# Unalome81/IEEE-802.11-OFDM-QPSK-Simulator

Hardware: AMD Instinct MI355X
Metric: OFDM symbols/sec (whole node) over BER-vs-SNR sweep; achieved HBM GB/s vs peak (higher is better)
Workload: dtype f32

## Files before the change

### ieee-802.11-ofdm-qpsk-simulator_amd/csrc/ofdm_rxcommon.h

```cpp
#pragma once
#include "ofdm_internal.h"

namespace ofdm {

struct TxSignSrc { uint32_t re, im; };
__host__ __device__ constexpr TxSignSrc tx_sign_src(const uint32_t (&w)[3], int m) {
    const uint32_t wd = w[(2 * m) >> 5];
    const int sh = (2 * m) & 31;
    return {(wd ^ (wd << 1)) << sh, wd << sh};
}
__host__ __device__ constexpr int tx_sign_tbl(int conv, int bin) { return (conv == OFDM_CONV_C && (bin & 1)) ? 0xD2 : 0x78; }
__host__ __device__ constexpr uint32_t bitop3_ref(uint32_t a, uint32_t b, uint32_t c, int tbl) {
    uint32_t o = 0u;
    for (int i = 0; i < 32; ++i) {
        const uint32_t idx = (((a >> i) & 1u) << 2) | (((b >> i) & 1u) << 1) | ((c >> i) & 1u);
        o |= (((uint32_t)tbl >> idx) & 1u) << i;
    }
    return o;
}
template <int CONV>
__host__ __device__ constexpr bool tx_sign_map_is_d10() {
    for (int bin = 0; bin < 64; ++bin) {
        const int m = data_index(bin);
        if (m < 0) continue;
// ... 127 lines not shown
struct SymState {
    float evm_pre;
    uint32_t be, ax;
    uint32_t d[3];
};

__device__ __forceinline__ void sym_init(SymState &st) {
    st.evm_pre = 0.f; st.be = 0u; st.ax = 0u; st.d[0] = st.d[1] = st.d[2] = 0u;
}
template <int KIND>
__device__ __forceinline__ float finish_evm(const SymState &st) { return KIND == 2 ? 4.0f * st.evm_pre : st.evm_pre; }

__device__ __forceinline__ uint32_t dbl_u32(uint32_t t) {
    uint32_t r;
    asm("v_add_u32_e32 %0, %1, %1" : "=v"(r) : "v"(t));
    return r;
}

template <bool DUMP, int R, int KIND, typename HF>
__device__ __forceinline__ void demap_sub(const float2 (&x)[64], uint32_t t, HF &&Hof, float2 *dump_eq, SymState &st) {
    uint32_t sm;
    asm volatile("v_mov_b32 %0, 0x80000000" : "=v"(sm));
    constexpr float cd = KIND == 2 ? 0.5f * INV_SQRT2 : INV_SQRT2;
    uint32_t em = 0u;
    static_for<0, 16>([&](auto kc) {
        constexpr int bin = 4 * decltype(kc)::value + R;
        constexpr int m = data_index(bin);
        if constexpr (m >= 0) {
            const EqOut<KIND> e = Hof(x[digit_rev4(bin)], std::integral_constant<int, bin>{});
            const uint32_t ti = t, tr = dbl_u32(t);
            t = dbl_u32(tr);
            const uint32_t ur = __builtin_amdgcn_bitop3_b32(__float_as_uint(e.u.x), tr, sm, 0x78);
            const uint32_t ui = __builtin_amdgcn_bitop3_b32(__float_as_uint(e.u.y), ti, sm, 0x78);
            float ex, ey;
            if constexpr (KIND == 0) {
                ex = __uint_as_float(ur) - cd;
                ey = __uint_as_float(ui) - cd;
            } else {
                ex = fmaf(__uint_as_float(ur), e.r, -cd);
                ey = fmaf(__uint_as_float(ui), e.r, -cd);
            }
            st.evm_pre = fmaf(ex, ex, fmaf(ey, ey, st.evm_pre));
            em = __builtin_amdgcn_alignbit(em, ur, 31);
            em = __builtin_amdgcn_alignbit(em, ui, 31);
            if constexpr (DUMP) {
                const float g = KIND == 0 ? 1.0f : KIND == 1 ? e.r : 2.0f * e.r;
                const float2 z = KIND == 0 ? e.u : make_float2(e.u.x * g, e.u.y * g);
                if (dump_eq) dump_eq[m] = z;
                const uint32_t pr = z.x > 0.f, pi = z.y > 0.f;
                constexpr int wi = (2 * m) >> 5;
                constexpr int s0 = 31 - ((2 * m) & 31), s1 = 31 - ((2 * m + 1) & 31);
                st.d[wi] |= ((pi ^ 1u) << s0) | ((pr ^ pi) << s1);
            }
        }
    });
    opaque(st.evm_pre);
    st.ax += __popc(em);
    st.be += __popc(em & 0x55555555u) + __popc((em ^ (em >> 1)) & 0x55555555u);
}

template <int BIN>
__device__ __forceinline__ EqOut<2> ls_equalise(float2 Y) {
    const float2 S = dpp_c<DPP_QUAD_BCAST0>(Y);
    EqOut<2> e;
    e.r = __builtin_amdgcn_rcpf(fmaf(S.x, S.x, S.y * S.y));
    e.u = cscale(cmulc(Y, S), (float)ltf_sign(BIN));
    return e;
}

template <typename F>
struct EqFn {
    F f;
    template <int R>
    __device__ __forceinline__ void prefetch(const float2 (&)[64]) {}
    template <typename B>
    __device__ __forceinline__ auto operator()(float2 Y, B b) { return f(Y, b); }
};
template <typename F>
__device__ __forceinline__ EqFn<F> eq_fn(F f) { return EqFn<F>{f}; }

struct FrameAcc {
    uint64_t errs = 0, frames = 0;
    int64_t pre_q = 0, dbpre_q = 0, dbpost_q = 0;
};

__device__ __forceinline__ int64_t q20_nonneg(float x) {
    const float v = __builtin_rintf(x * (float)OFDM_EVM_Q_SCALE);
    const float hi = __builtin_floorf(v * 0x1p-32f);
    const uint32_t lo = (uint32_t)fmaf(hi, -0x1p32f, v);
    return (int64_t)(((uint64_t)(uint32_t)hi << 32) | lo);
}
__device__ __forceinline__ int64_t q20_db(float db) {
    return (int64_t)(int32_t)__builtin_rintf(db * (float)OFDM_EVM_Q_SCALE);
}

__device__ __forceinline__ void frame_metrics(FrameAcc &acc, float fe_pre, uint32_t ferr, uint32_t fax) {
    constexpr float K = 3.01029995663981195214f, L96 = 6.58496250072115618146f;
    acc.errs = (uint64_t)ferr | ((uint64_t)fax << 32);
    acc.frames = (uint64_t)(ferr > 0u) | ((uint64_t)(fax > 0u) << 32);
    acc.pre_q = q20_nonneg(fe_pre);
    const float lg = K * (__builtin_amdgcn_logf(fe_pre) - L96);
    acc.dbpre_q = q20_db(fe_pre > 0.f ? fmaxf(lg, -400.0f) : -400.0f);
    acc.dbpost_q = fax > 0u ? q20_db(K * (__builtin_amdgcn_logf((float)fax) + (1.0f - L96))) : 0;
}

__device__ __forceinline__ void flush_lanes(const FrameAcc &acc, bool leader, unsigned long long *slots ) {
    if (leader) {
        atomicAdd(&slots[0], (unsigned long long)acc.errs);
        atomicAdd(&slots[1], (unsigned long long)acc.frames);
        atomicAdd(&slots[2], (unsigned long long)acc.pre_q);
        atomicAdd(&slots[3], (unsigned long long)acc.dbpre_q);
        atomicAdd(&slots[4], (unsigned long long)acc.dbpost_q);
    }
}

__device__ __forceinline__ int slot_term(const unsigned long long *s, int k, unsigned long long &v) {
    switch (k) {
        case 0: v = s[0] & 0xffffffffull; return OFDM_C_BIT_ERR;
        case 1: v = s[0] >> 32; return OFDM_C_EVM_POST_AXIS;
        case 2: v = s[1] & 0xffffffffull; return OFDM_C_FRAME_ERR;
        case 3: v = s[1] >> 32; return OFDM_C_EVMDB_POST_FINITE;
        case 4: v = s[2]; return OFDM_C_EVM_PRE_Q;
        case 5: v = s[3]; return OFDM_C_EVMDB_PRE_Q;
        default: v = s[4]; return OFDM_C_EVMDB_POST_Q;
    }
}

template <int S>
__device__ __forceinline__ void block_flush(const RxArgs &a, unsigned long long (*sacc)[S], int tid) {
    __syncthreads();
    for (int i = tid; i < a.n_snr * 7; i += blockDim.x) {
        const int q = i / 7, k = i % 7;
        unsigned long long v;
        const int ci = slot_term(sacc[q], k, v);
        if (v) atomicAdd(&a.counters[q * OFDM_NCOUNTERS + ci], v);
    }
    if (blockIdx.x == 0) {
        for (int q = tid; q < a.n_snr; q += blockDim.x) {
            unsigned long long *c = a.counters + q * OFDM_NCOUNTERS;
            atomicAdd(&c[OFDM_C_FRAMES], (unsigned long long)a.n_frames);
            atomicAdd(&c[OFDM_C_SYMBOLS], (unsigned long long)(2 * a.n_frames));
            atomicAdd(&c[OFDM_C_BITS], (unsigned long long)(192 * a.n_frames));
            atomicAdd(&c[OFDM_C_EVM_TERMS], (unsigned long long)(96 * a.n_frames));
        }
    }
}
template <int S>
__device__ __forceinline__ void block_flush(const RxArgs &a, unsigned long long (*sacc)[S]) {
    block_flush(a, sacc, (int)threadIdx.x);
}



template <int CONV, typename TA>
__device__ __forceinline__ void tx_symbol(const TA &a, int64_t sidx) {
    const uint64_t s = a.first_symbol + (uint64_t)sidx;
    uint32_t w[3];
    if (a.payload == OFDM_PAYLOAD_RANDOM) {
        const uint4 o = philox10((uint32_t)s, (uint32_t)(s >> 32), 0u, STREAM_BITS, a.k0, a.k1);
        w[0] = o.x; w[1] = o.y; w[2] = o.z;
    } else {
        const int r = (int)(s % (uint64_t)a.table_frames);
        w[0] = a.table[3 * r]; w[1] = a.table[3 * r + 1]; w[2] = a.table[3 * r + 2];
    }
    float2 X[64];
    static_for<0, 4>([&](auto gc) {
        constexpr int g = decltype(gc)::value;
        uint32_t wg[3] = {w[0], w[1], w[2]};
        opaque(wg[0]); opaque(wg[1]); opaque(wg[2]);
        static_for<0, 16>([&](auto pc) {
            constexpr int i = 16 * (decltype(pc)::value >> 2) + 4 * g + (decltype(pc)::value & 3);
            X[i] = tx_bin<CONV, i>(wg);
        });
        static_for<0, 4>([&](auto ic) { dif_stage1<true, 4 * g + decltype(ic)::value>(X); });
        sched_fence();
    });
    const uint32_t so = (uint32_t)sidx;
    [[maybe_unused]] const int64_t P = a.pitch;
    static_for<0, 4>([&](auto rc) {
        constexpr int R = decltype(rc)::value;
        dif_sub16<true, R>(X);
        static_for<0, 16>([&](auto nc) {
            constexpr int n = 4 * decltype(nc)::value + R;
            const float2 v = cscale(X[digit_rev4(n)], (n & 1) ? -1.0f / 64.0f : 1.0f / 64.0f);
            gst((gf2 *)(a.tx + (16 + n) * P), so, v);
            if constexpr (n >= 48) gst((gf2 *)(a.tx + (n - 48) * P), so, v);
        });
        sched_fence();
    });
    a.bits[so] = w[0];
    a.bits[P + so] = w[1];
    a.bits[2 * P + so] = w[2];
    a.bits[3 * P + so] = demap_word<0>(w);
    a.bits[4 * P + so] = demap_word<1>(w);
    a.bits[5 * P + so] = demap_word<2>(w);
    a.bits[6 * P + so] = demap_word<3>(w);
    uint32_t pw[3];
    pair_words(w, pw);
    a.bits[7 * P + so] = pw[0];
    a.bits[8 * P + so] = pw[1];
    a.bits[9 * P + so] = pw[2];
}

}
```

### ieee-802.11-ofdm-qpsk-simulator_amd/csrc/ofdm_rxpack.hip

```cpp
#include "ofdm_internal.h"
#include "ofdm_rxcommon.h"

#define OFDM_RX_PACK_WAVES 2
#define OFDM_RX_PACK_IDEAL_WAVES 3

namespace ofdm {

constexpr int PK_FRAMES = 64;
constexpr int PK_SYMS = 2 * PK_FRAMES;

typedef float f4v __attribute__((ext_vector_type(4)));
typedef __attribute__((address_space(3))) const f4v lcf4;
typedef unsigned int u2v __attribute__((ext_vector_type(2)));
typedef __attribute__((address_space(3))) const u2v lcu2;
typedef __attribute__((address_space(3))) f2v lf2;

constexpr int PACK_PF = 2;
constexpr int PACK_GEN_SPLIT = 2;
constexpr int PACK_FENCE_PAIRS = 2;

__host__ __device__ constexpr int rev16(int m) { return ((m & 3) << 2) | (m >> 2); }
__host__ __device__ constexpr int pos32(int k) { return (k & 1) ? 16 + rev16(k >> 1) : rev16(k >> 1); }

template <int K>
__device__ __forceinline__ float2 chan_bin(const float2 (&h)[4]) {
    float2 H = h[0];
    H = csub(H, twiddle<K * 1, false>(h[1]));
    H = cadd(H, twiddle<K * 2, false>(h[2]));
    return csub(H, twiddle<K * 3, false>(h[3]));
}

template <int HALF>
__device__ __forceinline__ void chan_pairs(const float2 (&h)[4], float4 *col) {
    static_for<12 * HALF, 12 * HALF + 12>([&](auto pc) {
        constexpr int p = decltype(pc)::value;
        constexpr int k = pair_bin(p);
        const float2 Hk = chan_bin<k>(h), Hm = chan_bin<64 - k>(h);
        col[p * PK_FRAMES] = make_float4(Hk.x, Hk.y, Hm.x, Hm.y);
        sched_fence();
    });
}

__device__ __forceinline__ void clean_spectrum(const RxArgs &a, int64_t s, float4 *spec_col ) {
    gcf2 *src = (gcf2 *)(a.tx + 16 * a.pitch + s);
    int P = (int)a.pitch;
    opaque(P);
    float2 x[64];
    static_for<0, 4>([&](auto gc) {
        constexpr int g = decltype(gc)::value;
        gcf2 *sp = src;
        opaque(sp);
        static_for<0, 16>([&](auto pc) {
            constexpr int n = 16 * (decltype(pc)::value >> 2) + 4 * g + (decltype(pc)::value & 3);
            const float2 v = gld(sp, n * P);
            x[n] = (n & 1) ? make_float2(-v.x, -v.y) : v;
        });
        static_for<0, 4>([&](auto ic) { dif_stage1<false, 4 * g + decltype(ic)::value>(x); });
        sched_fence();
    });
    auto store = [&](auto pc) {
        constexpr int p = decltype(pc)::value;
        constexpr int k = pair_bin(p);
        const float2 c0 = x[digit_rev4(k)], c1 = x[digit_rev4(64 - k)];
        spec_col[p * 2 * PK_FRAMES] = make_float4(c0.x, c0.y, c1.x, c1.y);
    };
    static_for<0, 4>([&](auto rc) { dif_sub16<false, decltype(rc)::value>(x); });
    static_for<0, PACK_PAIRS>(store);
}

template <int KIND, bool DUMP, bool WALK, int TBL>
__device__ __forceinline__ void demap_bin(float2 u, float r, uint32_t &t, float sx, float sy, uint32_t sm, float &evm,
                                          uint32_t &em, int m, float2 *dump_eq, uint32_t (&dbits)[3]) {
    constexpr float cd = KIND == 2 ? 0.5f * INV_SQRT2 : INV_SQRT2;
    uint32_t ur, ui;
    if constexpr (WALK) {
        const uint32_t ti = t, tr = dbl_u32(t);
        t = dbl_u32(tr);
        ur = __builtin_amdgcn_bitop3_b32(__float_as_uint(u.x), tr, sm, 0x78);
        ui = __builtin_amdgcn_bitop3_b32(__float_as_uint(u.y), ti, sm, 0x78);
    } else {
        ur = __builtin_amdgcn_bitop3_b32(__float_as_uint(u.x), __float_as_uint(sx), sm, TBL);
        ui = __builtin_amdgcn_bitop3_b32(__float_as_uint(u.y), __float_as_uint(sy), sm, TBL);
    }
    float ex, ey;
    if constexpr (KIND == 0) {
        ex = __uint_as_float(ur) - cd;
        ey = __uint_as_float(ui) - cd;
    } else {
        ex = fmaf(__uint_as_float(ur), r, -cd);
        ey = fmaf(__uint_as_float(ui), r, -cd);
    }
    evm = fmaf(ex, ex, fmaf(ey, ey, evm));
    em = __builtin_amdgcn_alignbit(em, ur, 31);
    em = __builtin_amdgcn_alignbit(em, ui, 31);
    if constexpr (DUMP) {
        const float g = KIND == 0 ? 1.0f : 2.0f * r;
        const float2 z = make_float2(u.x * g, u.y * g);
        if (dump_eq) dump_eq[m] = z;
        const uint32_t pr = z.x > 0.f, pi = z.y > 0.f;
        const int wi = (2 * m) >> 5, s0 = 31 - ((2 * m) & 31), s1 = 31 - ((2 * m + 1) & 31);
        dbits[wi] |= ((pi ^ 1u) << s0) | ((pr ^ pi) << s1);
    }
}

template <typename KS>
__device__ __forceinline__ Noise4 pack_noise(const PhiloxHead &hd, uint32_t c2, const KS &keys, uint32_t k1, float K) {
    uint4 o;
    if constexpr (std::is_same_v<KS, PhiloxKeysV>) o = philox10_c2(hd, c2, keys);
    else o = philox10_c2(hd, c2, keys, k1);
    return noise4_of(o, K);
}

typedef unsigned int u4v __attribute__((ext_vector_type(4)));
static_assert(sizeof(PhiloxWords) == sizeof(u4v), "one 16-byte read per block");
typedef __attribute__((address_space(3))) const u4v cwords;
__device__ __forceinline__ Noise4 pack_noise(const PhiloxMid &md, cwords *w, uint32_t k0, uint32_t k1, float K) {
    const u4v v = *w;
    return noise4_of(philox10_c2(md, v.x, v.y, v.z, k0, k1), K);
}
__device__ __forceinline__ Noise4 pack_noise(const PhiloxMid &md, lcu2 *w, lcu2 *q, uint32_t k0, uint32_t k1, float K) {
    const u2v v = *w, u = *q;
    return noise4_of(philox10_c2(md, v.x, v.y, u.x, u.y, k0, k1), K);
}

#ifdef OFDM_PACK_STAMPS
#include <cstdio>
static __device__ unsigned long long g_pack_stamps[4][8];
#define PK_STAMP(k)                                                                  \
    do {                                                                             \
        const unsigned long long t_ = __builtin_amdgcn_s_memtime();                  \
        st_acc[k] += t_ - st_t;                                                      \
        st_t = t_;                                                                   \
    } while (0)
#else
#define PK_STAMP(k) do { } while (0)
#endif

#define OFDM_RX_PACK_FADE_WAVES 2
#define PACK_SACC_SUB_LS 4
#define PACK_SACC_SUB 1
template <int KIND, int CONV, int CHAN, bool DUMP>
__global__ __launch_bounds__(256, KIND == 2 ? (CHAN == OFDM_CHAN_RAYLEIGH4 ? OFDM_RX_PACK_FADE_WAVES : OFDM_RX_PACK_WAVES)
                                            : OFDM_RX_PACK_IDEAL_WAVES) void rx_pack_kernel(RxArgs a) {
    constexpr bool FADE = CHAN == OFDM_CHAN_RAYLEIGH4;
    static_assert(!FADE || KIND == 2, "the packed Rayleigh receiver is the LS one");
    constexpr bool WLATE = KIND == 2 && !FADE;
    constexpr bool QW = KIND == 2 && !FADE;
    __shared__ __attribute__((aligned(16))) float4 spec[PACK_PAIRS][2][PK_FRAMES];
    __shared__ __attribute__((aligned(16))) float4 ce[PACK_PAIRS];
    __shared__ __attribute__((aligned(16))) float4 fce[FADE ? PACK_PAIRS : 1][FADE ? PK_FRAMES : 1];
    __shared__ __attribute__((aligned(8))) uint32_t truth[FADE ? 3 : 1][FADE ? PK_SYMS : 2];
    constexpr int SUBN = KIND != 2 ? PACK_SACC_SUB : FADE ? (PACK_SACC_SUB_LS < 4 ? PACK_SACC_SUB_LS : 4)
                                                      : PACK_SACC_SUB_LS;
    constexpr int SACC_XQ = 16;
    __shared__ unsigned long long sacc[OFDM_MAX_SNR][5];
    __shared__ unsigned long long sacx[SUBN > 1 ? SACC_XQ : 1][SUBN > 1 ? 5 * (SUBN - 1) : 1];
    auto slots = [&](int q, int ln) -> unsigned long long * {
        const int c = ln % SUBN;
        return SUBN > 1 && c > 0 && q < SACC_XQ ? &sacx[q][5 * (c - 1)] : sacc[q];
    };
    __shared__ __attribute__((aligned(16))) std::conditional_t<QW, u2v, u4v> wlds[PACK_BLOCKS];
    __shared__ __attribute__((aligned(8))) u2v qw[QW ? PACK_BLOCKS : 1][QW ? PK_FRAMES : 1];
    __shared__ uint32_t pf_dummy[64];
    __shared__ __attribute__((aligned(8))) float2 lds_keep[1];
    const int tid = threadIdx.x, lane = tid & 63;
    const int wv = __builtin_amdgcn_readfirstlane(tid >> 6);
#ifdef OFDM_PACK_STAMPS
    unsigned long long st_acc[8] = {0, 0, 0, 0, 0, 0, 0, 0};
    unsigned long long st_t = __builtin_amdgcn_s_memtime();
#endif
    for (int i = tid; i < a.n_snr * 5; i += blockDim.x) (&sacc[0][0])[i] = 0ull;
    if constexpr (SUBN > 1)
        for (int i = tid; i < SACC_XQ * 5 * (SUBN - 1); i += blockDim.x) (&sacx[0][0])[i] = 0ull;
    if constexpr (KIND == 2) {
        if (wv == 0) {
            float2 x[64];
            static_for<0, 64>([&](auto nc) {
                constexpr int n = decltype(nc)::value;
                const float2 v = a.ltf[n];
                x[n] = (n & 1) ? make_float2(-2.0f * v.x, -2.0f * v.y) : make_float2(2.0f * v.x, 2.0f * v.y);
            });
            fft64<false>(x);
            if (lane == 0) {
                static_for<0, PACK_PAIRS>([&](auto pc) {
                    constexpr int p = decltype(pc)::value;
                    constexpr int k = pair_bin(p);
                    const float2 c0 = x[digit_rev4(k)], c1 = x[digit_rev4(64 - k)];
                    ce[p] = make_float4(c0.x, c0.y, c1.x, c1.y);
                });
            }
        }
    }
    const int64_t n_groups = (a.n_frames + PK_FRAMES - 1) / PK_FRAMES;
    const int B = (int)gridDim.x, G = (int)n_groups, R = G / B, T = G - R * B;
    const int S = T > 0 ? max(1, min(4, B / T)) : 1;
    const int n_items = R * B + T * S;
    __shared__ int next_item;
    for (int w = blockIdx.x; w < n_items; w = __builtin_amdgcn_readfirstlane(next_item)) {
        const bool tail = w >= R * B;
        const int tw = tail ? w - R * B : 0;
        const int64_t grp = tail ? R * B + tw / S : w;
        const int sub = tail ? tw % S : 0, ns = tail ? S : 1;
        __syncthreads();
        PK_STAMP(0);
        const uint64_t fg = a.first_frame + (uint64_t)(grp * PK_FRAMES);
        const uint32_t row = (uint32_t)(fg >> 32) - (uint32_t)(a.first_frame >> 32);
        const bool uniform_hi = (uint32_t)((fg + (PK_FRAMES - 1)) >> 32) == (uint32_t)(fg >> 32) && row < 2u;
        int t = tid;
        opaque(t);
        if constexpr (QW) {
            if (uniform_hi) {
                const uint32_t flo = (uint32_t)fg + (uint32_t)(t & 63);
                const int s0 = (PACK_BLOCKS / 4) * wv;
#pragma unroll
                for (int i = 0; i < PACK_BLOCKS / 4; ++i) {
                    const uint2 qv = philox_qword(flo, a.philox_words[row * PACK_BLOCKS + s0 + i].y, a.k0);
                    u2v o; o.x = qv.x; o.y = qv.y;
                    qw[s0 + i][t & 63] = o;
                }
            }
        }
        using KArgs = const __attribute__((address_space(4))) RxArgs;
        KArgs *ap = (KArgs *)__builtin_amdgcn_kernarg_segment_ptr();
        asm volatile("" : "+s"(ap));
        const bool own_tx = ap->own.n_sym > 0;
        if (own_tx) {
            if (t >= PK_SYMS) {
                const int64_t sidx = grp * PK_SYMS + (t - PK_SYMS);
                if (sidx < ap->own.n_sym) {
                    if (ap->own_conv == OFDM_CONV_C) tx_symbol<OFDM_CONV_C>(ap->own, sidx);
                    else tx_symbol<OFDM_CONV_MATLAB>(ap->own, sidx);
                }
            }
            __syncthreads();
        }
        if (t < PK_SYMS) {
            clean_spectrum(a, grp * PK_SYMS + t, &spec[0][t & 1][t >> 1]);
        } else {
            const int j = t - PK_SYMS;
            if constexpr (FADE) {
                const uint32_t *src = a.bits + 7 * a.pitch + grp * PK_SYMS + j;
                truth[0][j] = src[0];
                truth[1][j] = src[a.pitch];
                truth[2][j] = src[2 * a.pitch];
            }
            if (j < 64) {
                int nx = 0;
                if (j == 0) nx = B + (int)atomicAdd(a.work, 1ull);
                nx = __builtin_amdgcn_readlane(nx, 0);
                if (j == 0) next_item = nx;
                if (nx < n_items && !own_tx && !WLATE) {
                    const int64_t ng = nx < R * B ? nx : R * B + (nx - R * B) / S;
#pragma unroll
                    for (int i = 0; i < 8; ++i) {
                        const int line = j + 64 * i;
                        const float2 *p = a.tx + (int64_t)(16 + (line >> 3)) * a.pitch + ng * PK_SYMS + (line & 7) * 16;
                        __builtin_amdgcn_global_load_lds((__attribute__((address_space(1))) void *)p,
                                                         (__attribute__((address_space(3))) void *)pf_dummy, 4, 0, 0);
                    }
                }
            }
            if (ap->nx.n_sym > 0 && sub == 0) {
                for (int64_t sidx = grp * PK_SYMS + j; sidx < ap->nx.n_sym; sidx += (int64_t)G * PK_SYMS) {
                    if (ap->nx_conv == OFDM_CONV_C) tx_symbol<OFDM_CONV_C>(ap->nx, sidx);
                    else tx_symbol<OFDM_CONV_MATLAB>(ap->nx, sidx);
                }
            }
            if (uniform_hi && j >= 64 && j < 64 + PACK_BLOCKS) {
                const u4v v = ((const u4v *)a.philox_words)[row * PACK_BLOCKS + (j - 64)];
                if constexpr (QW) { u2v o; o.x = v.x; o.y = v.z; wlds[j - 64] = o; }
                else wlds[j - 64] = v;
            }
            if constexpr (FADE) {
                const int fr = j & 63;
                const uint64_t ff = a.first_frame + (uint64_t)(grp * PK_FRAMES + fr);
                float2 h[4];
                channel_taps((uint32_t)ff, (uint32_t)(ff >> 32), a.k0, a.k1, h);
                if (j < 64) chan_pairs<0>(h, &fce[0][fr]);
                else chan_pairs<1>(h, &fce[0][fr]);
            }
        }
        PK_STAMP(1);
        __syncthreads();
        PK_STAMP(2);
        if constexpr (FADE) {
            for (int it = t; it < PACK_PAIRS * PK_FRAMES; it += 256) {
                const int p = it >> 6, fr = it & 63;
                const float4 H = fce[p][fr], c0 = spec[p][0][fr], c1 = spec[p][1][fr], e = ce[p];
                const float2 Hk = make_float2(H.x, H.y), Hm = make_float2(H.z, H.w);
                float2 u = cmul(Hk, make_float2(c0.x, c0.y)), v = cmul(Hm, make_float2(c0.z, c0.w));
                spec[p][0][fr] = make_float4(u.x, u.y, v.x, v.y);
                u = cmul(Hk, make_float2(c1.x, c1.y)); v = cmul(Hm, make_float2(c1.z, c1.w));
                spec[p][1][fr] = make_float4(u.x, u.y, v.x, v.y);
                u = cmul(Hk, make_float2(e.x, e.y)); v = cmul(Hm, make_float2(e.z, e.w));
                fce[p][fr] = make_float4(u.x, u.y, v.x, v.y);
            }
            __syncthreads();
        }
        PK_STAMP(3);
        const int64_t fl = grp * PK_FRAMES + lane;
        const bool valid = fl < a.n_frames;
        const uint64_t f = a.first_frame + (uint64_t)fl;
        auto snr_loop = [&](auto fastc) __attribute__((always_inline)) {
        constexpr bool FAST = decltype(fastc)::value;
        using WordsP = std::conditional_t<QW, lcu2, cwords> *;
        WordsP wtab = (WordsP)&wlds[0];
        for (int q = wv + 4 * sub; q < a.n_snr; q += 4 * ns) {
            if constexpr (WLATE) {
                if (wv == 2 && q + 4 * ns >= a.n_snr) {
                    const int nx = __builtin_amdgcn_readfirstlane(next_item);
                    using KArgsW = const __attribute__((address_space(4))) RxArgs;
                    KArgsW *apw = (KArgsW *)__builtin_amdgcn_kernarg_segment_ptr();
                    if (nx < n_items && apw->own.n_sym == 0) {
                        const int64_t ng = nx < R * B ? nx : R * B + (nx - R * B) / S;
                        int ln = lane;
                        opaque(ln);
#pragma unroll
                        for (int i = 0; i < 8; ++i) {
                            const int line = ln + 64 * i;
                            const float2 *p = a.tx + (int64_t)(16 + (line >> 3)) * a.pitch + ng * PK_SYMS + (line & 7) * 16;
                            __builtin_amdgcn_global_load_lds((__attribute__((address_space(1))) void *)p,
                                                             (__attribute__((address_space(3))) void *)pf_dummy, 4, 0, 0);
                        }
                    }
                }
            }
            uint32_t flo = (uint32_t)f, fhi = (uint32_t)(f >> 32);
            opaque(flo); opaque(fhi);
            const float sigma = a.sigma[q];
            const uint32_t qs = STREAM_NOISE | (uint32_t)(a.q_base + q);
            const PhiloxHead hd = philox_head(flo, fhi, qs, a.k1);
            const PhiloxMid md = philox_mid(hd);
            WordsP wt = wtab;
            lcu2 *qp = (lcu2 *)&qw[0][QW ? lane : 0];
            auto noise = [&](uint32_t blk, int slot, float Kn) __attribute__((always_inline)) {
                if constexpr (FAST && QW) return pack_noise(md, (lcu2 *)(wt + slot), qp + slot * PK_FRAMES, a.k0, a.k1, Kn);
                else if constexpr (FAST) return pack_noise(md, (cwords *)(wt + slot), a.k0, a.k1, Kn);
                else return pack_noise(hd, blk, a.k0, a.k1, Kn);
            };
            float2 z[64];
            float2 ee[PACK_PAIRS];
            lf2 *keep = (lf2 *)&lds_keep[0];
            opaque(keep);
            if constexpr (KIND == 2) {
                const float KE = noise_k(sigma * 1.41421356237309504880f);
                static_for<0, 4>([&](auto ic) {
                    constexpr int i = decltype(ic)::value;
                    uint32_t tg = 48u + 2 * i;
                    if constexpr (FAST) opaque(wt);
                    else opaque(tg);
                    if constexpr (FAST && QW) opaque(qp);
                    static_for<0, 2>([&](auto hc) {
                        constexpr int h = decltype(hc)::value;
                        const Noise4 lo = noise(tg + h, 2 * i + h, KE);
                        const Noise4 hi = noise(tg + 8 + h, 2 * i + 8 + h, KE);
                        constexpr int m = 4 * i + 2 * h;
                        z[m] = make_float2(lo.r0 * lo.c0, -(lo.r0 * lo.s0));
                        z[m + 1] = make_float2(lo.r1 * lo.c1, -(lo.r1 * lo.s1));
                        z[m + 16] = make_float2(hi.r0 * hi.c0, -(hi.r0 * hi.s0));
                        z[m + 17] = make_float2(hi.r1 * hi.c1, -(hi.r1 * hi.s1));
                    });
                    static_for<0, 4>([&](auto jc) {
                        constexpr int j = 4 * i + decltype(jc)::value;
                        const float2 u = z[j], v = z[j + 16];
                        z[j] = cadd(u, v);
                        z[j + 16] = twiddle<2 * j, false>(csub(u, v));
                    });
                    sched_fence();
                });
                dif4<false, 16, 0>(z);
                dif4<false, 16, 16>(z);
                static_for<0, PACK_PAIRS>([&](auto pc) {
                    constexpr int p = decltype(pc)::value;
                    constexpr int k = pair_bin(p);
                    const float2 P = z[pos32(k)], Qv = z[pos32(32 - k)];
                    const float2 F = make_float2(P.x + Qv.x, P.y - Qv.y);
                    const float2 H = twiddle<k, false>(make_float2(P.x - Qv.x, P.y + Qv.y));
                    ee[p] = make_float2(F.x + H.y, F.y - H.x);
                });
                sched_fence();
            }
            const float K = noise_k(sigma);
            float2 x[64];
            static_for<0, 4>([&](auto gc) {
                constexpr int g = decltype(gc)::value;
                uint32_t tg = 84u + g;
                if constexpr (FAST) opaque(wt);
                else opaque(tg);
                if constexpr (FAST && QW) opaque(qp);
                static_for<0, 4>([&](auto Qc) {
                    constexpr int Q = decltype(Qc)::value;
                    const Noise4 n0 = noise(tg + 4 * Q, 16 + g + 4 * Q, K);
                    const Noise4 n1 = noise(tg + 20 + 4 * Q, 32 + g + 4 * Q, K);
                    const float d0[4] = {n0.r0 * n0.c0, n0.r0 * n0.s0, n0.r1 * n0.c1, n0.r1 * n0.s1};
                    const float d1[4] = {n1.r0 * n1.c0, n1.r0 * n1.s0, n1.r1 * n1.c1, n1.r1 * n1.s1};
                    static_for<0, 4>([&](auto ic) {
                        constexpr int i = decltype(ic)::value;
                        x[16 * Q + 4 * g + i] = (i & 1) ? make_float2(-d0[i], -d1[i]) : make_float2(d0[i], d1[i]);
                    });
                    if constexpr (Q % PACK_GEN_SPLIT == PACK_GEN_SPLIT - 1 && Q < 3) sched_fence();
                });
                static_for<0, 4>([&](auto ic) { dif_stage1<false, 4 * g + decltype(ic)::value>(x); });
                sched_fence();
            });
            float2 *deq0 = nullptr, *deq1 = nullptr;
            uint32_t *dbit0 = nullptr, *dbit1 = nullptr;
            if constexpr (DUMP) {
                if (valid) {
                    const int64_t r0 = ((int64_t)q * a.dump_frames + fl) * 2;
                    deq0 = a.dump_eq + r0 * 48; deq1 = deq0 + 48;
                    dbit0 = a.dump_bits + r0 * 3; dbit1 = dbit0 + 3;
                }
            }
            uint32_t db0[3] = {0u, 0u, 0u}, db1[3] = {0u, 0u, 0u};
            lcf4 *sp = (lcf4 *)&spec[0][0][lane];
            lcu2 *tw = (lcu2 *)&truth[0][FADE ? 2 * lane : 0];
            lcf4 *fp = (lcf4 *)&fce[0][FADE ? lane : 0];
            opaque(sp);
            if constexpr (FADE) opaque(tw);
            if constexpr (FADE) opaque(fp);
            uint32_t sm;
            asm volatile("v_mov_b32 %0, 0x80000000" : "=v"(sm));
            float evm = 0.f;
            uint32_t em = 0u, be = 0u, ax = 0u, t0 = 0u, t1 = 0u;
            constexpr int PF = KIND == 2 && !FADE ? PACK_PF : 0;
            f4v pc0[PF + 1], pc1[PF + 1];
            float4 pe4[PF + 1];
            auto load_pair = [&](auto pc) {
                constexpr int p = decltype(pc)::value;
                if constexpr (p < PACK_PAIRS) {
                    constexpr int slot = p % (PF + 1);
                    pc0[slot] = sp[p * 2 * PK_FRAMES];
                    pc1[slot] = sp[(p * 2 + 1) * PK_FRAMES];
                    if constexpr (KIND == 2) {
                        if constexpr (FADE) {
                            const f4v v = fp[p * PK_FRAMES];
                            pe4[slot] = make_float4(v.x, v.y, v.z, v.w);
                        } else {
                            pe4[slot] = ce[p];
                        }
                    }
                }
            };
            if constexpr (PF > 0) static_for<0, PF>(load_pair);
            auto pair = [&](auto pc) {
                constexpr int p = decltype(pc)::value;
                constexpr int k = pair_bin(p), k2 = 64 - k;
                if constexpr (FADE && (p & 7) == 0) {
                    const u2v tt = tw[(p >> 3) * (PK_SYMS / 2)];
                    t0 = tt.x; t1 = tt.y;
                }
                if constexpr (PF > 0) load_pair(std::integral_constant<int, p + PF>{});
                constexpr int slot = p % (PF + 1);
                const float2 Zk = x[digit_rev4(k)], Zm = x[digit_rev4(k2)];
                const float2 A = make_float2(Zk.x + Zm.x, Zk.y - Zm.y), B = make_float2(Zk.x - Zm.x, Zk.y + Zm.y);
                if constexpr (PF == 0) load_pair(pc);
                const f4v c0 = pc0[slot], c1 = pc1[slot];
                const float2 y0k = make_float2(fmaf(0.5f, A.x, c0.x), fmaf(0.5f, A.y, c0.y));
                const float2 y0m = make_float2(fmaf(0.5f, A.x, c0.z), fmaf(-0.5f, A.y, c0.w));
                const float2 y1k = make_float2(fmaf(0.5f, B.y, c1.x), fmaf(-0.5f, B.x, c1.y));
                const float2 y1m = make_float2(fmaf(0.5f, B.y, c1.z), fmaf(0.5f, B.x, c1.w));
                float2 u0k, u0m, u1k, u1m;
                float rk = 0.f, rm = 0.f;
                if constexpr (KIND == 2) {
                    const float ex = ee[p].x, ey = ee[p].y;
                    const float4 e4 = pe4[slot];
                    const float2 Sk = make_float2(fmaf(0.5f, ex, e4.x), fmaf(0.5f, ey, e4.y));
                    const float2 Sm = make_float2(fmaf(0.5f, ex, e4.z), fmaf(-0.5f, ey, e4.w));
                    rk = __builtin_amdgcn_rcpf(fmaf(Sk.x, Sk.x, Sk.y * Sk.y));
                    rm = __builtin_amdgcn_rcpf(fmaf(Sm.x, Sm.x, Sm.y * Sm.y));
                    u0k = cscale(cmulc(y0k, Sk), (float)ltf_sign(k));
                    u1k = cscale(cmulc(y1k, Sk), (float)ltf_sign(k));
                    u0m = cscale(cmulc(y0m, Sm), (float)ltf_sign(k2));
                    u1m = cscale(cmulc(y1m, Sm), (float)ltf_sign(k2));
                } else {
                    constexpr float cs = (CONV == OFDM_CONV_C && (k & 1)) ? -1.0f : 1.0f;
                    u0k = cscale(y0k, cs); u0m = cscale(y0m, cs); u1k = cscale(y1k, cs); u1m = cscale(y1m, cs);
                }
                constexpr int TBL = (CONV == OFDM_CONV_C && (k & 1)) ? 0xD2 : 0x78;
                demap_bin<KIND, DUMP, FADE, TBL>(u0k, rk, t0, c0.x, c0.y, sm, evm, em, data_index(k), deq0, db0);
                demap_bin<KIND, DUMP, FADE, TBL>(u0m, rm, t0, c0.z, c0.w, sm, evm, em, data_index(k2), deq0, db0);
                demap_bin<KIND, DUMP, FADE, TBL>(u1k, rk, t1, c1.x, c1.y, sm, evm, em, data_index(k), deq1, db1);
                demap_bin<KIND, DUMP, FADE, TBL>(u1m, rm, t1, c1.z, c1.w, sm, evm, em, data_index(k2), deq1, db1);
                if constexpr ((p & 3) == 3) {
                    ax += __popc(em);
                    be += __popc(em & 0x55555555u) + __popc((em ^ (em >> 1)) & 0x55555555u);
                    em = 0u;
                }
                opaque(evm);
                if constexpr (p % PACK_FENCE_PAIRS == PACK_FENCE_PAIRS - 1) sched_fence();
            };
            dif_sub16<false, 0>(x);
            static_for<0, 6>(pair);
            sched_fence();
            dif_sub16<false, 2>(x);
            static_for<6, 13>(pair);
            sched_fence();
            dif_sub16<false, 1>(x);
            dif_sub16<false, 3>(x);
            static_for<13, 24>(pair);
            if constexpr (DUMP) {
                if (dbit0) {
                    dbit0[0] = db0[0]; dbit0[1] = db0[1]; dbit0[2] = db0[2];
                    dbit1[0] = db1[0]; dbit1[1] = db1[1]; dbit1[2] = db1[2];
                }
            }
            FrameAcc acc;
            frame_metrics(acc, KIND == 2 ? 4.0f * evm : evm, be, ax);
            flush_lanes(acc, valid, slots(q, lane));
        }
        };
        if (uniform_hi) snr_loop(std::true_type{});
        else snr_loop(std::false_type{});
        PK_STAMP(4);
    }
    if constexpr (SUBN > 1) {
        __syncthreads();
        for (int i = tid; i < min(a.n_snr, SACC_XQ) * 5; i += 256) {
            const int q = i / 5, k = i % 5;
            unsigned long long v = sacc[q][k];
#pragma unroll
            for (int c = 1; c < SUBN; ++c) v += sacx[q][5 * (c - 1) + k];
            sacc[q][k] = v;
        }
    }
    block_flush(a, sacc, tid);
    PK_STAMP(5);
#ifdef OFDM_PACK_STAMPS
    if (lane == 0)
        for (int k = 0; k < 6; ++k) atomicAdd(&g_pack_stamps[wv][k], st_acc[k]);
#endif
}

template <int KIND, int CONV, int CHAN = OFDM_CHAN_AWGN>
static void launch_pack_t(hipStream_t st, const RxArgs &a, bool dump, unsigned grid) {
    if (dump) hipLaunchKernelGGL((rx_pack_kernel<KIND, CONV, CHAN, true>), dim3(grid), dim3(256), 0, st, a);
    else hipLaunchKernelGGL((rx_pack_kernel<KIND, CONV, CHAN, false>), dim3(grid), dim3(256), 0, st, a);
#ifdef OFDM_PACK_STAMPS
    unsigned long long hs[4][8];
    if (hipStreamSynchronize(st) == hipSuccess && hipMemcpyFromSymbol(hs, HIP_SYMBOL(g_pack_stamps), sizeof hs) == hipSuccess) {
        static const char *names[6] = {"item-top barrier", "prologue work", "prologue barrier", "faded spectra",
                                       "SNR loop", "block flush"};
        for (int w : {0, 2}) {
            double tot = 0;
            for (int k = 0; k < 6; ++k) tot += (double)hs[w][k];
            fprintf(stderr, "pack stamp wave %d:", w);
            for (int k = 0; k < 6; ++k) fprintf(stderr, " %s %.2f%%;", names[k], 100.0 * (double)hs[w][k] / tot);
            fprintf(stderr, "\n");
        }
    }
#endif
}

template <const void *(*K)()>
static int pack_grid(int64_t n_frames, int device) {
    const int64_t need = (n_frames + PK_FRAMES - 1) / PK_FRAMES;
    int per_cu = 0, cus = 0;
    if (hipOccupancyMaxActiveBlocksPerMultiprocessor(&per_cu, K(), 256, 0) != hipSuccess || per_cu < 1) per_cu = 1;
    if (hipDeviceGetAttribute(&cus, hipDeviceAttributeMultiprocessorCount, device) != hipSuccess || cus < 1) cus = 256;
    const int64_t cap = (int64_t)per_cu * cus;
    const int64_t g = need < cap ? need : cap;
    return (int)(g < 1 ? 1 : g);
}

#ifdef OFDM_RXPACK_IDEAL_TU
static const void *ideal_kernel() { return reinterpret_cast<const void *>(&rx_pack_kernel<0, OFDM_CONV_C, OFDM_CHAN_AWGN, false>); }

void launch_rx_pack_ideal(hipStream_t st, const RxArgs &a, const ofdm_cfg &cfg, bool dump, unsigned grid) {
    if (cfg.conv == OFDM_CONV_C) launch_pack_t<0, OFDM_CONV_C>(st, a, dump, grid);
    else launch_pack_t<0, OFDM_CONV_MATLAB>(st, a, dump, grid);
}

int rx_pack_ideal_grid(int64_t n_frames, int device) { return pack_grid<ideal_kernel>(n_frames, device); }
#else
bool rx_pack_applies(const ofdm_cfg &cfg) {
    if (cfg.noise != OFDM_NOISE_REAL) return false;
    if (cfg.channel == OFDM_CHAN_RAYLEIGH4) return cfg.est == OFDM_EST_LS;
    return cfg.channel == OFDM_CHAN_AWGN;
}

void pack_philox_table(uint32_t k0, uint32_t k1, uint32_t frame_hi, PhiloxWords (&out)[2][PACK_BLOCKS]) {
    for (int r = 0; r < 2; ++r)
        for (int s = 0; s < PACK_BLOCKS; ++s) out[r][s] = philox_words(frame_hi + (uint32_t)r, pack_block(s), k0, k1);
}

void launch_rx_pack(hipStream_t st, const RxArgs &a, const ofdm_cfg &cfg, bool dump, unsigned grid) {
    if (cfg.est == OFDM_EST_LS && cfg.channel == OFDM_CHAN_RAYLEIGH4)
        launch_pack_t<2, OFDM_CONV_C, OFDM_CHAN_RAYLEIGH4>(st, a, dump, grid);
    else if (cfg.est == OFDM_EST_LS) {
        if (cfg.conv == OFDM_CONV_C) launch_pack_t<2, OFDM_CONV_C>(st, a, dump, grid);
        else launch_pack_t<2, OFDM_CONV_MATLAB>(st, a, dump, grid);
    }
    else launch_rx_pack_ideal(st, a, cfg, dump, grid);
}

static const void *ls_kernel() { return reinterpret_cast<const void *>(&rx_pack_kernel<2, OFDM_CONV_C, OFDM_CHAN_AWGN, false>); }
static const void *fade_kernel() {
    return reinterpret_cast<const void *>(&rx_pack_kernel<2, OFDM_CONV_C, OFDM_CHAN_RAYLEIGH4, false>);
}

int rx_pack_grid(const ofdm_cfg &cfg, int64_t n_frames, int device) {
    if (cfg.est != OFDM_EST_LS) return rx_pack_ideal_grid(n_frames, device);
    return cfg.channel == OFDM_CHAN_RAYLEIGH4 ? pack_grid<fade_kernel>(n_frames, device)
                                              : pack_grid<ls_kernel>(n_frames, device);
}
#endif

}
```

Measured before the change: 13.20 billion.

## Compute pack prologue into registers before barrier and fuse own-tx spectrum in-register

```diff
diff --git a/ieee-802.11-ofdm-qpsk-simulator_amd/csrc/ofdm_rxcommon.h b/ieee-802.11-ofdm-qpsk-simulator_amd/csrc/ofdm_rxcommon.h
--- a/ieee-802.11-ofdm-qpsk-simulator_amd/csrc/ofdm_rxcommon.h
+++ b/ieee-802.11-ofdm-qpsk-simulator_amd/csrc/ofdm_rxcommon.h
@@ -303,8 +303,11 @@
 
 
 
-template <int CONV, typename TA>
-__device__ __forceinline__ void tx_symbol(const TA &a, int64_t sidx) {
+struct TxKeepNone {
+    template <typename N> __device__ __forceinline__ void operator()(N, float2) const {}
+};
+template <int CONV, typename TA, typename Keep = TxKeepNone>
+__device__ __forceinline__ void tx_symbol(const TA &a, int64_t sidx, Keep keep = Keep{}) {
     const uint64_t s = a.first_symbol + (uint64_t)sidx;
     uint32_t w[3];
     if (a.payload == OFDM_PAYLOAD_RANDOM) {
@@ -335,6 +338,7 @@
             constexpr int n = 4 * decltype(nc)::value + R;
             const float2 v = cscale(X[digit_rev4(n)], (n & 1) ? -1.0f / 64.0f : 1.0f / 64.0f);
             gst((gf2 *)(a.tx + (16 + n) * P), so, v);
+            keep(std::integral_constant<int, n>{}, v);
             if constexpr (n >= 48) gst((gf2 *)(a.tx + (n - 48) * P), so, v);
         });
         sched_fence();
diff --git a/ieee-802.11-ofdm-qpsk-simulator_amd/csrc/ofdm_rxpack.hip b/ieee-802.11-ofdm-qpsk-simulator_amd/csrc/ofdm_rxpack.hip
--- a/ieee-802.11-ofdm-qpsk-simulator_amd/csrc/ofdm_rxpack.hip
+++ b/ieee-802.11-ofdm-qpsk-simulator_amd/csrc/ofdm_rxpack.hip
@@ -41,7 +41,20 @@
     });
 }
 
-__device__ __forceinline__ void clean_spectrum(const RxArgs &a, int64_t s, float4 *spec_col ) {
+template <typename Put>
+__device__ __forceinline__ void spectrum_tail(float2 (&x)[64], Put put) {
+    auto store = [&](auto pc) {
+        constexpr int p = decltype(pc)::value;
+        constexpr int k = pair_bin(p);
+        const float2 c0 = x[digit_rev4(k)], c1 = x[digit_rev4(64 - k)];
+        put(pc, make_float4(c0.x, c0.y, c1.x, c1.y));
+    };
+    static_for<0, 4>([&](auto rc) { dif_sub16<false, decltype(rc)::value>(x); });
+    static_for<0, PACK_PAIRS>(store);
+}
+
+template <typename Put>
+__device__ __forceinline__ void clean_spectrum(const RxArgs &a, int64_t s, Put put) {
     gcf2 *src = (gcf2 *)(a.tx + 16 * a.pitch + s);
     int P = (int)a.pitch;
     opaque(P);
@@ -58,14 +71,17 @@
         static_for<0, 4>([&](auto ic) { dif_stage1<false, 4 * g + decltype(ic)::value>(x); });
         sched_fence();
     });
-    auto store = [&](auto pc) {
-        constexpr int p = decltype(pc)::value;
-        constexpr int k = pair_bin(p);
-        const float2 c0 = x[digit_rev4(k)], c1 = x[digit_rev4(64 - k)];
-        spec_col[p * 2 * PK_FRAMES] = make_float4(c0.x, c0.y, c1.x, c1.y);
-    };
-    static_for<0, 4>([&](auto rc) { dif_sub16<false, decltype(rc)::value>(x); });
-    static_for<0, PACK_PAIRS>(store);
+    spectrum_tail(x, put);
+}
+
+template <typename Put>
+__device__ __forceinline__ void clean_spectrum_of(float2 (&x)[64], Put put) {
+    static_for<0, 4>([&](auto gc) {
+        constexpr int g = decltype(gc)::value;
+        static_for<0, 4>([&](auto ic) { dif_stage1<false, 4 * g + decltype(ic)::value>(x); });
+        sched_fence();
+    });
+    spectrum_tail(x, put);
 }
 
 template <int KIND, bool DUMP, bool WALK, int TBL>
@@ -145,7 +161,10 @@
     constexpr bool FADE = CHAN == OFDM_CHAN_RAYLEIGH4;
     static_assert(!FADE || KIND == 2, "the packed Rayleigh receiver is the LS one");
     constexpr bool WLATE = KIND == 2 && !FADE;
+    constexpr bool PRE = KIND == 2 && !FADE;
+    constexpr bool OWN_REG = PRE;
     constexpr bool QW = KIND == 2 && !FADE;
+    static_assert(PRE == QW, "the carried philox_qword values are the LS AWGN receiver's");
     __shared__ __attribute__((aligned(16))) float4 spec[PACK_PAIRS][2][PK_FRAMES];
     __shared__ __attribute__((aligned(16))) float4 ce[PACK_PAIRS];
     __shared__ __attribute__((aligned(16))) float4 fce[FADE ? PACK_PAIRS : 1][FADE ? PK_FRAMES : 1];
@@ -201,30 +220,20 @@
         const int tw = tail ? w - R * B : 0;
         const int64_t grp = tail ? R * B + tw / S : w;
         const int sub = tail ? tw % S : 0, ns = tail ? S : 1;
-        __syncthreads();
-        PK_STAMP(0);
+        if constexpr (!PRE) {
+            __syncthreads();
+            PK_STAMP(0);
+        }
         const uint64_t fg = a.first_frame + (uint64_t)(grp * PK_FRAMES);
         const uint32_t row = (uint32_t)(fg >> 32) - (uint32_t)(a.first_frame >> 32);
         const bool uniform_hi = (uint32_t)((fg + (PK_FRAMES - 1)) >> 32) == (uint32_t)(fg >> 32) && row < 2u;
         int t = tid;
         opaque(t);
-        if constexpr (QW) {
-            if (uniform_hi) {
-                const uint32_t flo = (uint32_t)fg + (uint32_t)(t & 63);
-                const int s0 = (PACK_BLOCKS / 4) * wv;
-#pragma unroll
-                for (int i = 0; i < PACK_BLOCKS / 4; ++i) {
-                    const uint2 qv = philox_qword(flo, a.philox_words[row * PACK_BLOCKS + s0 + i].y, a.k0);
-                    u2v o; o.x = qv.x; o.y = qv.y;
-                    qw[s0 + i][t & 63] = o;
-                }
-            }
-        }
         using KArgs = const __attribute__((address_space(4))) RxArgs;
         KArgs *ap = (KArgs *)__builtin_amdgcn_kernarg_segment_ptr();
         asm volatile("" : "+s"(ap));
         const bool own_tx = ap->own.n_sym > 0;
-        if (own_tx) {
+        if (own_tx && !OWN_REG) {
             if (t >= PK_SYMS) {
                 const int64_t sidx = grp * PK_SYMS + (t - PK_SYMS);
                 if (sidx < ap->own.n_sym) {
@@ -234,8 +243,54 @@
             }
             __syncthreads();
         }
-        if (t < PK_SYMS) {
-            clean_spectrum(a, grp * PK_SYMS + t, &spec[0][t & 1][t >> 1]);
+        u2v pq[QW ? PACK_BLOCKS / 4 : 1];
+        if constexpr (QW) {
+            const uint32_t qrow = uniform_hi ? row : 0u;
+            const uint32_t flo = (uint32_t)fg + (uint32_t)(t & 63);
+            const int s0 = (PACK_BLOCKS / 4) * wv;
+#pragma unroll
+            for (int i = 0; i < PACK_BLOCKS / 4; ++i) {
+                const uint2 qv = philox_qword(flo, a.philox_words[qrow * PACK_BLOCKS + s0 + i].y, a.k0);
+                pq[i].x = qv.x; pq[i].y = qv.y;
+            }
+        }
+        const bool spectra = PRE ? wv < 2 : t < PK_SYMS;
+        auto top_barrier = [&]() __attribute__((always_inline)) {
+            PK_STAMP(0);
+            __syncthreads();
+            PK_STAMP(1);
+        };
+        if (spectra) {
+            if constexpr (PRE) {
+                float4 pv[PACK_PAIRS];
+                auto hold = [&](auto pc, float4 v) { pv[decltype(pc)::value] = v; };
+                if (OWN_REG && own_tx) {
+                    const int64_t sidx = grp * PK_SYMS + t;
+                    float2 x[64];
+                    auto keep = [&](auto nc, float2 v) {
+                        constexpr int n = decltype(nc)::value;
+                        opaque(v.x); opaque(v.y);
+                        x[n] = (n & 1) ? make_float2(-v.x, -v.y) : v;
+                    };
+                    if (sidx >= ap->own.n_sym) {
+                        static_for<0, 64>([&](auto nc) { x[decltype(nc)::value] = make_float2(0.f, 0.f); });
+                    } else if (ap->own_conv == OFDM_CONV_C) {
+                        tx_symbol<OFDM_CONV_C>(ap->own, sidx, keep);
+                    } else {
+                        tx_symbol<OFDM_CONV_MATLAB>(ap->own, sidx, keep);
+                    }
+                    clean_spectrum_of(x, hold);
+                } else {
+                    clean_spectrum(a, grp * PK_SYMS + t, hold);
+                }
+                top_barrier();
+                float4 *col = &spec[0][t & 1][t >> 1];
+                static_for<0, PACK_PAIRS>([&](auto pc) { col[decltype(pc)::value * 2 * PK_FRAMES] = pv[decltype(pc)::value]; });
+            } else {
+                float4 *col = &spec[0][t & 1][t >> 1];
+                clean_spectrum(a, grp * PK_SYMS + t,
+                               [&](auto pc, float4 v) { col[decltype(pc)::value * 2 * PK_FRAMES] = v; });
+            }
         } else {
             const int j = t - PK_SYMS;
             if constexpr (FADE) {
@@ -244,11 +299,14 @@
                 truth[1][j] = src[a.pitch];
                 truth[2][j] = src[2 * a.pitch];
             }
+            u4v wrow = {0u, 0u, 0u, 0u};
+            int nxr = 0;
             if (j < 64) {
                 int nx = 0;
                 if (j == 0) nx = B + (int)atomicAdd(a.work, 1ull);
                 nx = __builtin_amdgcn_readlane(nx, 0);
-                if (j == 0) next_item = nx;
+                if constexpr (PRE) nxr = nx;
+                else if (j == 0) next_item = nx;
                 if (nx < n_items && !own_tx && !WLATE) {
                     const int64_t ng = nx < R * B ? nx : R * B + (nx - R * B) / S;
 #pragma unroll
@@ -268,7 +326,7 @@
             }
             if (uniform_hi && j >= 64 && j < 64 + PACK_BLOCKS) {
                 const u4v v = ((const u4v *)a.philox_words)[row * PACK_BLOCKS + (j - 64)];
-                if constexpr (QW) { u2v o; o.x = v.x; o.y = v.z; wlds[j - 64] = o; }
+                if constexpr (PRE) wrow = v;
                 else wlds[j - 64] = v;
             }
             if constexpr (FADE) {
@@ -279,10 +337,27 @@
                 if (j < 64) chan_pairs<0>(h, &fce[0][fr]);
                 else chan_pairs<1>(h, &fce[0][fr]);
             }
-        }
-        PK_STAMP(1);
+            if constexpr (PRE) {
+                top_barrier();
+                if (j == 0) next_item = nxr;
+                if (uniform_hi && j >= 64 && j < 64 + PACK_BLOCKS) {
+                    u2v o; o.x = wrow.x; o.y = wrow.z;
+                    wlds[j - 64] = o;
+                }
+            }
+        }
+        if constexpr (PRE) {
+            if (uniform_hi) {
+                const int s0 = (PACK_BLOCKS / 4) * wv;
+#pragma unroll
+                for (int i = 0; i < PACK_BLOCKS / 4; ++i) qw[s0 + i][t & 63] = pq[i];
+            }
+            PK_STAMP(2);
+        } else {
+            PK_STAMP(1);
+        }
         __syncthreads();
-        PK_STAMP(2);
+        PK_STAMP(PRE ? 3 : 2);
         if constexpr (FADE) {
             for (int it = t; it < PACK_PAIRS * PK_FRAMES; it += 256) {
                 const int p = it >> 6, fr = it & 63;
@@ -297,7 +372,7 @@
             }
             __syncthreads();
         }
-        PK_STAMP(3);
+        if constexpr (!PRE) PK_STAMP(3);
         const int64_t fl = grp * PK_FRAMES + lane;
         const bool valid = fl < a.n_frames;
         const uint64_t f = a.first_frame + (uint64_t)fl;
@@ -539,8 +614,11 @@
 #ifdef OFDM_PACK_STAMPS
     unsigned long long hs[4][8];
     if (hipStreamSynchronize(st) == hipSuccess && hipMemcpyFromSymbol(hs, HIP_SYMBOL(g_pack_stamps), sizeof hs) == hipSuccess) {
-        static const char *names[6] = {"item-top barrier", "prologue work", "prologue barrier", "faded spectra",
-                                       "SNR loop", "block flush"};
+        static const char *const names_pre[6] = {"pre-work", "top barrier", "stores", "second barrier", "SNR loop",
+                                                 "block flush"};
+        static const char *const names_old[6] = {"item-top barrier", "prologue work", "prologue barrier",
+                                                 "faded spectra", "SNR loop", "block flush"};
+        const char *const *names = KIND == 2 && CHAN != OFDM_CHAN_RAYLEIGH4 ? names_pre : names_old;
         for (int w : {0, 2}) {
             double tot = 0;
             for (int k = 0; k < 6; ++k) tot += (double)hs[w][k];
```

New measurement: 13.32 billion, median of 6. Within noise of the previous version (+0.9%).

## Software-pipeline LDS Philox word loads ahead of noise regions

Applied to the files above, without the earlier changes.

```diff
diff --git a/ieee-802.11-ofdm-qpsk-simulator_amd/csrc/ofdm_rxpack.hip b/ieee-802.11-ofdm-qpsk-simulator_amd/csrc/ofdm_rxpack.hip
--- a/ieee-802.11-ofdm-qpsk-simulator_amd/csrc/ofdm_rxpack.hip
+++ b/ieee-802.11-ofdm-qpsk-simulator_amd/csrc/ofdm_rxpack.hip
@@ -18,6 +18,18 @@
 constexpr int PACK_PF = 2;
 constexpr int PACK_GEN_SPLIT = 2;
 constexpr int PACK_FENCE_PAIRS = 2;
+
+constexpr int PACK_REGIONS = 12;
+static_assert(PACK_GEN_SPLIT == 2, "a data group's noise regions are its halves");
+__host__ __device__ constexpr int noise_slot(int r, int j) {
+    return r < 4 ? 2 * r + (j >> 1) + 8 * (j & 1) : 16 + ((r - 4) >> 1) + 4 * (2 * ((r - 4) & 1) + (j >> 1)) + 16 * (j & 1);
+}
+#ifndef OFDM_PACK_AHEAD
+#define OFDM_PACK_AHEAD 0x222222222222
+#endif
+__host__ __device__ constexpr int pack_ahead(int r) {
+    return r >= 0 && r < PACK_REGIONS ? (int)(((unsigned long long)OFDM_PACK_AHEAD >> (4 * r)) & 3u) : 0;
+}
 
 __host__ __device__ constexpr int rev16(int m) { return ((m & 3) << 2) | (m >> 2); }
 __host__ __device__ constexpr int pos32(int k) { return (k & 1) ? 16 + rev16(k >> 1) : rev16(k >> 1); }
@@ -118,9 +130,13 @@
     const u4v v = *w;
     return noise4_of(philox10_c2(md, v.x, v.y, v.z, k0, k1), K);
 }
-__device__ __forceinline__ Noise4 pack_noise(const PhiloxMid &md, lcu2 *w, lcu2 *q, uint32_t k0, uint32_t k1, float K) {
-    const u2v v = *w, u = *q;
+__device__ __forceinline__ Noise4 pack_noise(const PhiloxMid &md, u2v v, u2v u, uint32_t k0, uint32_t k1, float K) {
     return noise4_of(philox10_c2(md, v.x, v.y, u.x, u.y, k0, k1), K);
+}
+
+__device__ __forceinline__ void warm_line(const float2 *p, uint32_t *lds_dummy ) {
+    const uint32_t m = (uint32_t)(uintptr_t)(__attribute__((address_space(3))) uint32_t *)lds_dummy;
+    asm volatile("s_mov_b32 m0, %1\n\ts_nop 0\n\tglobal_load_lds_dword %0, off" : : "v"(p), "s"(m) : "m0");
 }
 
 #ifdef OFDM_PACK_STAMPS
@@ -319,11 +335,38 @@
                         for (int i = 0; i < 8; ++i) {
                             const int line = ln + 64 * i;
                             const float2 *p = a.tx + (int64_t)(16 + (line >> 3)) * a.pitch + ng * PK_SYMS + (line & 7) * 16;
-                            __builtin_amdgcn_global_load_lds((__attribute__((address_space(1))) void *)p,
-                                                             (__attribute__((address_space(3))) void *)pf_dummy, 4, 0, 0);
+                            warm_line(p, pf_dummy);
                         }
                     }
                 }
+            }
+            WordsP wt = wtab;
+            lcu2 *qp = (lcu2 *)&qw[0][QW ? lane : 0];
+            constexpr bool AHEAD = FAST && QW;
+            u2v ow[2][4], oq[2][4];
+            auto fetch = [&](auto rc, auto lo, auto hi) __attribute__((always_inline)) {
+                constexpr int r = decltype(rc)::value, LO = decltype(lo)::value, HI = decltype(hi)::value;
+                static_for<0, 4>([&](auto jc) {
+                    constexpr int j = decltype(jc)::value, s = noise_slot(r, j);
+                    if constexpr (LO <= 2 && 2 <= HI) ow[r & 1][j] = *(lcu2 *)(wt + s);
+                    if constexpr (LO <= 1 && 1 <= HI) oq[r & 1][j] = qp[s * PK_FRAMES];
+                });
+            };
+            auto region_top = [&](auto rc) __attribute__((always_inline)) {
+                constexpr int r = decltype(rc)::value;
+                if constexpr (AHEAD) {
+                    constexpr int own = pack_ahead(r), nxt = pack_ahead(r + 1);
+                    if constexpr (r >= 0 && own < 2) fetch(rc, std::integral_constant<int, own + 1>{}, std::integral_constant<int, 2>{});
+                    if constexpr (nxt > 0) {
+                        fetch(std::integral_constant<int, r + 1>{}, std::integral_constant<int, 3 - nxt>{},
+                              std::integral_constant<int, 2>{});
+                        sched_fence();
+                    }
+                }
+            };
+            if constexpr (AHEAD && pack_ahead(0) > 0) {
+                opaque(wt); opaque(qp);
+                region_top(std::integral_constant<int, -1>{});
             }
             uint32_t flo = (uint32_t)f, fhi = (uint32_t)(f >> 32);
             opaque(flo); opaque(fhi);
@@ -331,10 +374,10 @@
             const uint32_t qs = STREAM_NOISE | (uint32_t)(a.q_base + q);
             const PhiloxHead hd = philox_head(flo, fhi, qs, a.k1);
             const PhiloxMid md = philox_mid(hd);
-            WordsP wt = wtab;
-            lcu2 *qp = (lcu2 *)&qw[0][QW ? lane : 0];
-            auto noise = [&](uint32_t blk, int slot, float Kn) __attribute__((always_inline)) {
-                if constexpr (FAST && QW) return pack_noise(md, (lcu2 *)(wt + slot), qp + slot * PK_FRAMES, a.k0, a.k1, Kn);
+            if constexpr (AHEAD && pack_ahead(0) > 0 && pack_ahead(1) > 0) asm volatile("" : : "s"(sigma));
+            auto noise = [&](uint32_t blk, int slot, float Kn, auto rc, auto jc) __attribute__((always_inline)) {
+                if constexpr (AHEAD) return pack_noise(md, ow[decltype(rc)::value & 1][decltype(jc)::value],
+                                                       oq[decltype(rc)::value & 1][decltype(jc)::value], a.k0, a.k1, Kn);
                 else if constexpr (FAST) return pack_noise(md, (cwords *)(wt + slot), a.k0, a.k1, Kn);
                 else return pack_noise(hd, blk, a.k0, a.k1, Kn);
             };
@@ -350,10 +393,11 @@
                     if constexpr (FAST) opaque(wt);
                     else opaque(tg);
                     if constexpr (FAST && QW) opaque(qp);
+                    region_top(ic);
                     static_for<0, 2>([&](auto hc) {
                         constexpr int h = decltype(hc)::value;
-                        const Noise4 lo = noise(tg + h, 2 * i + h, KE);
-                        const Noise4 hi = noise(tg + 8 + h, 2 * i + 8 + h, KE);
+                        const Noise4 lo = noise(tg + h, 2 * i + h, KE, ic, std::integral_constant<int, 2 * h>{});
+                        const Noise4 hi = noise(tg + 8 + h, 2 * i + 8 + h, KE, ic, std::integral_constant<int, 2 * h + 1>{});
                         constexpr int m = 4 * i + 2 * h;
                         z[m] = make_float2(lo.r0 * lo.c0, -(lo.r0 * lo.s0));
                         z[m + 1] = make_float2(lo.r1 * lo.c1, -(lo.r1 * lo.s1));
@@ -390,8 +434,10 @@
                 if constexpr (FAST && QW) opaque(qp);
                 static_for<0, 4>([&](auto Qc) {
                     constexpr int Q = decltype(Qc)::value;
-                    const Noise4 n0 = noise(tg + 4 * Q, 16 + g + 4 * Q, K);
-                    const Noise4 n1 = noise(tg + 20 + 4 * Q, 32 + g + 4 * Q, K);
+                    using RC = std::integral_constant<int, 4 + 2 * g + (Q >> 1)>;
+                    if constexpr ((Q & 1) == 0) region_top(RC{});
+                    const Noise4 n0 = noise(tg + 4 * Q, 16 + g + 4 * Q, K, RC{}, std::integral_constant<int, 2 * (Q & 1)>{});
+                    const Noise4 n1 = noise(tg + 20 + 4 * Q, 32 + g + 4 * Q, K, RC{}, std::integral_constant<int, 2 * (Q & 1) + 1>{});
                     const float d0[4] = {n0.r0 * n0.c0, n0.r0 * n0.s0, n0.r1 * n0.c1, n0.r1 * n0.s1};
                     const float d1[4] = {n1.r0 * n1.c0, n1.r0 * n1.s0, n1.r1 * n1.c1, n1.r1 * n1.s1};
                     static_for<0, 4>([&](auto ic) {
```

After: 13.26 billion before, 13.38 billion after (median of 6 runs). No clear change (+0.9%).
